# ntampellini/FIRECODE

Measured on AMD Instinct MI355X. Metric: conformer-pair RMSD alignments/s, higher is better.
Workload: dtype f64

## Files before the change

firecode_amd/csrc/fc_items.h:

```cpp
#pragma once

#include <algorithm>
#include <cstdint>
#include <utility>
#include <vector>

#if defined(__HIPCC__) || defined(__CUDACC__)
#define FC_ITEMS_HD __host__ __device__
#else
#define FC_ITEMS_HD
#endif

namespace fc {

FC_ITEMS_HD inline int64_t global_block(int64_t local_block, int64_t rank, int64_t world) {
  return local_block * world + ((local_block & 1) ? (world - 1 - rank) : rank);
}
inline int64_t local_block_count(int64_t n_gblocks, int64_t rank, int64_t world) {
  int64_t n = 0;
  while (global_block(n, rank, world) < n_gblocks) ++n;
  return n;
}

constexpr uint64_t kItemFirstHalf = 1ull << 31, kItemSecondHalf = 1ull << 63;
constexpr int kItemChunkShift = 58, kItemChunkMax = 16;
FC_ITEMS_HD inline int64_t item_tile(uint64_t it) { return (int64_t)(it & 0x7fffffffull); }
FC_ITEMS_HD inline int64_t item_block(uint64_t it) { return (int64_t)((it >> 32) & 0x3ffffffull); }
FC_ITEMS_HD inline int item_blocks(uint64_t it) { return (int)((it >> kItemChunkShift) & 15ull) + 1; }

struct ItemPlan {
  int64_t N = 0, rank = 0, world = 1;
  int64_t row_block = 128, tc = 64;
  int64_t NT = 0, n_lblocks = 0;
  bool halves = false;
  int64_t tail = 0;
  bool real_columns_only = false;
  int64_t chunk = 1;
  bool tail_order = true;
};

template <class F>
inline void item_units(uint64_t it, const ItemPlan &p, F visit) {
  const int64_t jt = item_tile(it), lb = item_block(it), j0 = jt * p.tc, tpb = p.row_block / 16;
  int64_t it_first = 0, it_last = tpb * item_blocks(it);
  if (it & kItemFirstHalf) it_last = tpb / 2;
  if (it & kItemSecondHalf) it_first = tpb / 2;
  const int64_t i0 = global_block(lb, p.rank, p.world) * p.row_block;
  if (i0 >= p.N || j0 + p.tc - 1 <= i0) return;
  for (int64_t t = it_first; t < it_last; ++t) {
    const int64_t ib = global_block(lb + t / tpb, p.rank, p.world) * p.row_block + (t % tpb) * 16;
    if (ib >= p.N) break;
    if (j0 + p.tc - 1 <= ib) break;
    for (int64_t cs = 0; cs < p.tc / 16; ++cs) {
      if (j0 + (cs + 1) * 16 - 1 <= ib) continue;
      if (j0 + cs * 16 >= p.N) continue;
      visit(ib, j0 + cs * 16);
    }
  }
}

inline std::vector<uint64_t> build_items(const ItemPlan &p) {
  std::vector<uint64_t> items;
  if (p.row_block % p.tc != 0) return items;
  const int64_t r = p.row_block / p.tc;
  const int64_t nt = p.real_columns_only ? std::min(p.NT, (p.N + p.tc - 1) / p.tc) : p.NT;
  auto first_tile = [&](int64_t l) { return r * global_block(l, p.rank, p.world); };
  auto n_single = [&](int64_t l) { return std::max<int64_t>(0, nt - first_tile(l)); };
  int64_t n_chunked = 0;
  if (p.chunk > 1) {
    int64_t kept = 0;
    n_chunked = p.n_lblocks;
    while (n_chunked > 0 && kept < (p.tail_order ? 3 : 1) * p.tail) kept += n_single(--n_chunked);
    if (n_chunked < 2) n_chunked = 0;
  }
  const int64_t chunk = std::min<int64_t>(p.chunk, kItemChunkMax);
  for (int64_t l = 0; l < n_chunked; l += chunk) {
    const uint64_t more = (uint64_t)(std::min(chunk, n_chunked - l) - 1);
    for (int64_t jt = first_tile(l); jt < nt; ++jt) items.push_back((more << kItemChunkShift) | ((uint64_t)l << 32) | (uint64_t)jt);
  }
  const size_t single0 = items.size();
  for (int64_t l = n_chunked; l < p.n_lblocks; ++l)
    for (int64_t jt = first_tile(l); jt < nt; ++jt) items.push_back(((uint64_t)l << 32) | (uint64_t)jt);
  if (p.chunk > 1 && p.tail_order) {
    auto cost = [&](uint64_t it) {
      int64_t n = 0;
      item_units(it, p, [&](int64_t, int64_t) { ++n; });
      return n;
    };
    std::vector<std::pair<int64_t, uint64_t>> keyed;
    for (size_t k = single0; k < items.size(); ++k) keyed.emplace_back(-cost(items[k]), items[k]);
    std::stable_sort(keyed.begin(), keyed.end(), [](const auto &a, const auto &b) { return a.first < b.first; });
    for (size_t k = single0; k < items.size(); ++k) items[k] = keyed[k - single0].second;
  }
  if (p.halves && p.tail > 0 && (int64_t)items.size() > 4 * p.tail && (int64_t)(items.size() - single0) >= p.tail) {
    std::vector<uint64_t> halves;
    for (int64_t k = (int64_t)items.size() - p.tail; k < (int64_t)items.size(); ++k) {
      halves.push_back(items[(size_t)k] | kItemFirstHalf);
      halves.push_back(items[(size_t)k] | kItemSecondHalf);
    }
    items.resize(items.size() - (size_t)p.tail);
    items.insert(items.end(), halves.begin(), halves.end());
  }
  return items;
}

}
```

firecode_amd/csrc/fc_kabsch.hip:

```cpp
#include <type_traits>

#include "fc_internal.h"
#include <vector>
#include "fc_kabsch_math.h"

#include <algorithm>
#include <cstdlib>

namespace fc {

__global__ void __launch_bounds__(256)
k_prep(const double *__restrict__ coords, int64_t N, int64_t A_all, const int32_t *__restrict__ sel,
       int64_t A, int center, int64_t Npad, double *__restrict__ Xs, double *__restrict__ G,
       double *__restrict__ Xa, unsigned long long *__restrict__ gmax_bits,
       const int32_t *__restrict__ conf_idx) {
  const int64_t n = (int64_t)blockIdx.x * blockDim.x + threadIdx.x;
  if (n >= Npad) return;
  for (int64_t a = A; a < ((A + 3) & ~(int64_t)3); ++a) {
    Xs[(a * 3 + 0) * Npad + n] = 0.0;
    Xs[(a * 3 + 1) * Npad + n] = 0.0;
    Xs[(a * 3 + 2) * Npad + n] = 0.0;
  }
  if (n >= N) {
    for (int64_t a = 0; a < A; ++a) {
// ... 333 lines not shown
  if (!INV && pi[p] == pj[p]) {
    rmsd[p] = 0.0;
    maxdev[p] = 0.0;
    if (Rout)
      for (int k = 0; k < 9; ++k) Rout[p * 9 + k] = (k % 4 == 0) ? 1.0 : 0.0;
    return;
  }
  pair_exact_aos<INV>(Xa, A, pi[p], pj[p], r, m, Rout ? Rout + p * 9 : nullptr);
  rmsd[p] = r;
  maxdev[p] = m;
}

__global__ void __launch_bounds__(256)
k_matrix_exact(const double *__restrict__ Xs, int64_t N, int64_t Npad, int A,
               double *__restrict__ rmsd, double *__restrict__ maxdev) {
  const int lane = threadIdx.x & 63;
  const int64_t wave = ((int64_t)blockIdx.x * blockDim.x + threadIdx.x) >> 6;
  const int64_t NT = Npad >> 6;
  const int64_t i = wave / NT;
  const int64_t jt = wave % NT;
  if (i >= N) return;
  if (jt * 64 + 63 <= i) return;
  const int64_t j = jt * 64 + lane;
  if (j >= N || j <= i) return;
  double r, m;
  pair_exact(Xs, Npad, A, i, j, r, m);
  rmsd[i * N + j] = r;
  maxdev[i * N + j] = m;
}

__device__ __forceinline__ void push_pairs(uint64_t m, bool may, unsigned i, unsigned j,
                                           uint64_t *__restrict__ pairq, unsigned long long Q,
                                           unsigned long long *__restrict__ counters, int lane) {
  if (m == 0) return;
#ifdef FC_ABLATE_PUSH
  return;
#endif
  unsigned long long base = 0;
  if (lane == 0) base = atomicAdd(&counters[6], (unsigned long long)__popcll(m));
  base = __shfl(base, 0);
  if (may) {
    const unsigned long long slot = base + (unsigned long long)__popcll(m & ((1ull << lane) - 1ull));
    if (slot < Q) pairq[slot] = ((uint64_t)i << 32) | (uint64_t)j;
  }
}

#ifndef FC_REFINE_ROUNDS
#define FC_REFINE_ROUNDS 4
#endif
constexpr int kStagePairs = 48;
constexpr int kStageWords = 24;
constexpr size_t kStageBytes = kStagePairs * 8 + kStageWords * 4 + 8;
constexpr int64_t kCompleteRowChunk = 2;

#ifndef FC_STAGE_PAIRS_F32
#define FC_STAGE_PAIRS_F32 384
#endif
constexpr int kStagePairsF32 = FC_STAGE_PAIRS_F32;
constexpr int kStageWordsF32 = 128;
constexpr size_t kStageBytesF32 = kStagePairsF32 * 8 + kStageWordsF32 * 4 + 16 + 32 * 4;

template <int CAP = kStagePairs>
__device__ __forceinline__ void stage_pairs(uint64_t m, bool may, unsigned i, unsigned j,
                                            uint64_t *__restrict__ sq, unsigned *__restrict__ scnt,
                                            uint64_t *__restrict__ pairq, unsigned long long Q,
                                            unsigned long long *__restrict__ counters, int lane) {
  if (m == 0) return;
#ifdef FC_ABLATE_PUSH
  return;
#endif
#ifdef FC_ABLATE_STAGE
  if (lane == 0) scnt[2] = (unsigned)__popcll(m);
  return;
#endif
  const unsigned n = (unsigned)__popcll(m);
  unsigned base = 0;
  if (lane == 0) base = atomicAdd(scnt, n);
  base = (unsigned)__builtin_amdgcn_readfirstlane((int)base);
  if (base + n <= (unsigned)CAP) {
    if (may) sq[base + (unsigned)__popcll(m & ((1ull << lane) - 1ull))] = ((uint64_t)i << 32) | (uint64_t)j;
  } else {
#ifndef FC_ABLATE_OVERFLOW
    push_pairs(m, may, i, j, pairq, Q, counters, lane);
#endif
  }
}

template <int WCAP>
__device__ __forceinline__ void stage_pairs_wave(uint64_t m, bool may, unsigned i, unsigned j, uint64_t *__restrict__ sq_wave,
                                                 int &n_staged, uint64_t *__restrict__ pairq, unsigned long long Q,
                                                 unsigned long long *__restrict__ counters, int lane) {
  if (m == 0) return;
  const int n = (int)__popcll(m);
  if (n_staged + n <= WCAP) {
    if (may) sq_wave[n_staged + (int)__popcll(m & ((1ull << lane) - 1ull))] = ((uint64_t)i << 32) | (uint64_t)j;
    n_staged += n;
  } else {
    push_pairs(m, may, i, j, pairq, Q, counters, lane);
  }
}

__device__ __forceinline__ void flush_pairs_wave32(const uint32_t *__restrict__ sq_wave, int n_staged, unsigned i0, unsigned j0,
                                                   uint64_t *__restrict__ pairq, unsigned long long Q,
                                                   unsigned long long *__restrict__ counters, int lane) {
  if (n_staged == 0) return;
  unsigned long long base = 0;
// ... 74 lines not shown
        qz = lds[(a * 3 + 2) * 64 + lane];
      } else {
        qx = xq[(int64_t)(a * 3 + 0) * Npad];
        qy = xq[(int64_t)(a * 3 + 1) * Npad];
        qz = xq[(int64_t)(a * 3 + 2) * Npad];
      }
      const double *__restrict__ px = xp + (int64_t)(a * 3 + 0) * Npad;
      const double *__restrict__ py = xp + (int64_t)(a * 3 + 1) * Npad;
      const double *__restrict__ pz = xp + (int64_t)(a * 3 + 2) * Npad;
#pragma unroll
      for (int k = 0; k < TI; ++k) {
        const double x = px[k], y = py[k], z = pz[k];
        acc[k][0] = fma(x, qx, acc[k][0]);
        acc[k][1] = fma(x, qy, acc[k][1]);
        acc[k][2] = fma(x, qz, acc[k][2]);
        acc[k][3] = fma(y, qx, acc[k][3]);
        acc[k][4] = fma(y, qy, acc[k][4]);
        acc[k][5] = fma(y, qz, acc[k][5]);
        acc[k][6] = fma(z, qx, acc[k][6]);
        acc[k][7] = fma(z, qy, acc[k][7]);
        acc[k][8] = fma(z, qz, acc[k][8]);
      }
    }
#pragma unroll
    for (int k = 0; k < TI; ++k) {
      const int64_t i = ib + k;
      const double Gp = G[i];
      bool may = kabsch_may_be_below<ENANT>(acc[k], Gp + Gq, A_thr2);
      may = may && (j > i) && (j < N) && (i < N);
      const uint64_t word = __ballot(may);
      push_pairs(word, may, (unsigned)i, (unsigned)j, pairq, Q, counters, lane);
      if (lane == 0 && i < N) {
        const int64_t lrow = (int64_t)(lb * IB) + (int64_t)it * TI + k;
        bits[lrow * W + jt] = word;
        if (word) {
          const unsigned long long slot = atomicAdd(&counters[4], 1ull);
          cand[slot] = (uint32_t)(lrow * W + jt);
        }
      }
    }
  }
}

typedef double d4_t __attribute__((ext_vector_type(4)));

template <int NW, int MODE = 0, int TC = 64, bool EIG = false, bool ENANT = false>
__global__ void __launch_bounds__(NW * 64, 2)
k_simbits_screen_mfma(const double *__restrict__ Xs, const double *__restrict__ G, int64_t N,
                      int64_t Npad, int A, double A_thr2, int IB, int64_t rank, int64_t world,
                      uint64_t *__restrict__ bits, int64_t W, uint32_t *__restrict__ cand,
                      unsigned long long *__restrict__ counters, uint64_t *__restrict__ pairq,
                      unsigned long long Q, const uint64_t *__restrict__ item_table, unsigned long long n_items,
                      double *__restrict__ rmsd_out = nullptr, const unsigned long long *__restrict__ gate = nullptr,
                      double *__restrict__ maxdev_out = nullptr) {
  static_assert(!EIG || MODE == 2, "EIG: the complete alignments");
  static_assert(!ENANT || MODE == 0, "ENANT: the screen only");
  constexpr bool VALUES = MODE != 0;
  constexpr int NT = MODE == 2 ? 1 : 2;
  static_assert(TC == 64 || ((TC == 32 || TC == 16) && MODE == 2), "column tiles: 64, or 32 / 16 for the complete alignments");
  constexpr int NU = (TC / 16) / NT;
  constexpr int KPR = TC == 64 ? 2 : 4;
  constexpr int SST = 2048 / TC;
  constexpr int CST = TC == 64 ? 256 : 128;
  auto koff = [](int sl) { return TC == 16 ? (sl >> 1) * 384 + (sl & 1) * 64 : sl * (12 * TC); };
  if (gate != nullptr && *gate == 0ull) return;
  extern __shared__ double lds[];
  const int tid = threadIdx.x;
  const int lane = tid & 63;
  const int wv = __builtin_amdgcn_readfirstlane(tid >> 6);
  const int KS = (A + 3) >> 2;
  double *__restrict__ ldsG = lds + (TC == 16 ? ((KS + 1) >> 1) * 384 : KS * 12 * TC);
  uint64_t *__restrict__ stageQ = reinterpret_cast<uint64_t *>(ldsG + TC + IB);
  uint32_t *__restrict__ stageW = reinterpret_cast<uint32_t *>(stageQ + kStagePairs);
  unsigned *__restrict__ stageN = reinterpret_cast<unsigned *>(stageW + kStageWords);
#ifdef FC_TIMELINE
  unsigned long long *tl = MODE == 2 ? reinterpret_cast<unsigned long long *>(bits) : reinterpret_cast<unsigned long long *>(rmsd_out);
  constexpr bool TL = MODE == 0 || MODE == 2;
#endif
  const unsigned long long b = blockIdx.x;
  if (b >= n_items) return;
#ifdef FC_TIMELINE
  if (TL && tl && tid == 0) {
    tl[(size_t)b * 4] = wall_clock64();
    tl[(size_t)b * 4 + 3] = b;
  }
#endif
  int64_t jt, lb;
  int it_first = 0, it_last = IB >> 4;
  if (item_table != nullptr) {
    const uint64_t it = item_table[b];
    lb = item_block(it);
    jt = item_tile(it);
    if constexpr (MODE == 2) it_last = (IB >> 4) * item_blocks(it);
    if (it & kItemFirstHalf) it_last = IB >> 5;
    if (it & kItemSecondHalf) it_first = IB >> 5;
  } else {
    const int64_t NT = Npad / TC;
    jt = (int64_t)(b % (unsigned long long)NT);
    lb = (int64_t)(b / (unsigned long long)NT);
  }
  const int64_t j0 = jt * TC;
  const int64_t i0 = global_block(lb, rank, world) * IB;
  if (i0 >= N) return;
  if (j0 + TC - 1 <= i0) return;
  uint32_t *__restrict__ sq32_wave = reinterpret_cast<uint32_t *>(stageQ) + wv * (kStagePairs * 2 / NW);
  int n_staged32 = 0;
  (void)sq32_wave;
  (void)n_staged32;

  {
    const int n_runs = TC == 64 ? KS * 6 : (TC == 32 ? KS * 3 : ((KS + 1) >> 1) * 3);
    const int cs_l = TC == 64 ? lane >> 4 : lane >> 5, k1_l = TC == 64 ? (lane >> 3) & 1 : (lane >> 3) & 3, c15_l = (lane & 7) * 2;
    for (int q = wv; q < n_runs; q += NW) {
      const int sc = TC == 64 ? q >> 1 : q, kh = TC == 64 ? q & 1 : 0;
      const int sg = sc / 3, c = sc - sg * 3;
      int a = sg * 4 + kh * 2 + k1_l;
      if (TC == 16) {
        a = (sg * 2 + cs_l) * 4 + k1_l;
        a = a < KS * 4 ? a : KS * 4 - 1;
      }
      const double *src = Xs + (int64_t)(a * 3 + c) * Npad + j0 + (TC == 16 ? 0 : cs_l * 16) + c15_l;
      __builtin_amdgcn_global_load_lds((const __attribute__((address_space(1))) void *)src,
                                       (__attribute__((address_space(3))) void *)(lds + q * 128), 16, 0, 0);
    }
    for (int idx = tid; idx < TC + IB; idx += NW * 64) {
      const int64_t g = idx < TC ? j0 + idx : i0 + (idx - TC);
      ldsG[idx] = g < Npad ? G[g] : 0.0;
    }
    if (tid < kStagePairs) stageQ[tid] = ~0ull;
    if (tid < kStageWords) stageW[tid] = ~0u;
    if (tid < 2) stageN[tid] = 0u;
    __syncthreads();
#ifdef FC_TIMELINE
    if (TL && tl && tid == 0) tl[(size_t)b * 4 + 1] = wall_clock64();
#endif
  }
  const int kq = lane >> 4, l15 = lane & 15;
  const int lcol = MODE == 2 ? 4 * (l15 & 3) + (l15 >> 2) : l15;
  const int boff = (kq / KPR) * 128 + (kq % KPR) * 16 + lcol;
  uint16_t *bits16 = reinterpret_cast<uint16_t *>(bits);

  double a0[3], a1[3], a2[3];
  int pre_it = -1;
  const int tpb = IB >> 4;
  auto tile_row = [&](int it_) -> int64_t {
    if constexpr (MODE == 2) {
      const int k = it_ / tpb;
      return global_block(lb + k, rank, world) * IB + (int64_t)(it_ - k * tpb) * 16;
    } else {
      return i0 + (int64_t)it_ * 16;
    }
  };
  auto row_offsets = [&](int it_, unsigned (&vo)[3]) {
    const int64_t ib_ = tile_row(it_);
#pragma unroll
    for (int c = 0; c < 3; ++c) vo[c] = (unsigned)(((int64_t)(kq * 3 + c) * Npad + ib_ + l15) * 8);
  };
  auto fetch_a_at = [&](double (&a)[3], unsigned (&vo)[3], int sx) {
    const int sl = sx < KS ? sx : KS - 1;
    const char *__restrict__ xs_s = reinterpret_cast<const char *>(Xs + (int64_t)sl * 12 * Npad);
#pragma unroll
    for (int c = 0; c < 3; ++c) {
      asm volatile("" : "+v"(vo[c]));
      a[c] = *reinterpret_cast<const double *>(xs_s + vo[c]);
    }
  };

  for (int it = it_first + wv; it < it_last; it += NW) {
    const int64_t ib = tile_row(it);
    if (ib >= N) break;
    if (j0 + TC - 1 <= ib) break;
    const int64_t lrow0 = lb * IB + (int64_t)it * 16;
    double Gp_row = 0.0;
    if constexpr (MODE == 2) Gp_row = G[ib + l15];
    (void)Gp_row;
    unsigned nz = 0;
    unsigned voff[3];
    row_offsets(it, voff);

#pragma unroll 1
    for (int half = 0; half < NU; ++half) {
      const int cs0 = half * NT;
      if (j0 + (cs0 + NT) * 16 - 1 <= ib) {
        if (!VALUES && lane < 16 && ib + lane < N) {
          bits16[((lrow0 + lane) * W + jt) * 4 + cs0] = 0;
          bits16[((lrow0 + lane) * W + jt) * 4 + cs0 + 1] = 0;
        }
        continue;
      }
      if constexpr (MODE == 2) {
        if (j0 + cs0 * 16 >= N) continue;
      }
      d4_t acc[NT][9];

      const double *__restrict__ lb0 = lds + cs0 * SST + boff;
      double b0[NT][3], b1[NT][3];
      const int KSe = KS;
      auto fetch_a = [&](double (&a)[3], int sx) {
        fetch_a_at(a, voff, sx);
      };
      auto fetch_b = [&](double (&b)[NT][3], int sx) {
        const int sl = sx < KS ? sx : KS - 1;
        const double *__restrict__ lb_s = lb0 + koff(sl);
#pragma unroll
        for (int t = 0; t < NT; ++t)
#pragma unroll
          for (int c = 0; c < 3; ++c) b[t][c] = lb_s[c * CST + t * SST];
      };
      auto mma = [&](const double (&a)[3], const double (&b)[NT][3], auto first_) {
        constexpr bool first = decltype(first_)::value;
#pragma unroll
        for (int x = 0; x < 3; ++x)
#pragma unroll
          for (int y = 0; y < 3; ++y)
#pragma unroll
            for (int t = 0; t < NT; ++t) {
              const d4_t c_in = first ? d4_t{0.0, 0.0, 0.0, 0.0} : acc[t][x * 3 + y];
              acc[t][x * 3 + y] = MODE == 2 ? __builtin_amdgcn_mfma_f64_16x16x4f64(b[t][y], a[x], c_in, 0, 0, 0)
                                            : __builtin_amdgcn_mfma_f64_16x16x4f64(a[x], b[t][y], c_in, 0, 0, 0);
            }
      };
      if (pre_it != it) {
        fetch_a_at(a0, voff, 0);
        fetch_a_at(a1, voff, 1);
        fetch_a_at(a2, voff, 2);
      }
      fetch_b(b0, 0);
      fetch_b(b1, 1);
#define FC_KSTEP(AX, BX, U)             \
  if (sgrp + (U) < KSe) {               \
    mma(AX, BX, std::false_type{});     \
    fetch_a(AX, sgrp + (U) + 3);        \
    fetch_b(BX, sgrp + (U) + 2);        \
  }
      mma(a0, b0, std::true_type{});
      fetch_a(a0, 3);
      fetch_b(b0, 2);
      for (int sgrp = 1; sgrp < KSe; sgrp += 6) {
        FC_KSTEP(a1, b1, 0)
        FC_KSTEP(a2, b0, 1)
        FC_KSTEP(a0, b1, 2)
        FC_KSTEP(a1, b0, 3)
        FC_KSTEP(a2, b1, 4)
        FC_KSTEP(a0, b0, 5)
      }
#undef FC_KSTEP
      {
        const bool same_tile = half < NU - 1 && !(MODE == 2 && j0 + (cs0 + NT) * 16 >= N);
        const int nit = same_tile ? it : it + NW;
        bool more = same_tile;
        if (!same_tile && nit < it_last) {
          const int64_t nib = tile_row(nit);
          more = nib < N && !(j0 + TC - 1 <= nib);
        }
        if (more) {
          unsigned vn[3];
          row_offsets(nit, vn);
          fetch_a_at(a0, vn, 0);
          fetch_a_at(a1, vn, 1);
          fetch_a_at(a2, vn, 2);
          pre_it = nit;
        } else {
          pre_it = -1;
        }
      }
      const int n32 = (int)N, ib32 = (int)ib;
#pragma unroll
      for (int t = 0; t < NT; ++t) {
        const int cs = cs0 + t;
        const int j = (int)j0 + cs * 16 + l15;
        const double Gq = ldsG[cs * 16 + l15];
        uint64_t mr[4] = {0, 0, 0, 0};
        if (MODE == 2) {
          const int i = ib32 + l15;
          const int jb = (int)j0 + cs * 16 + 4 * kq;
          const double Gp = Gp_row;
          double nR[4][9];
          bool ok4[4];
          double msdA4[4] = {0.0, 0.0, 0.0, 0.0};
          {
            double B4[4][9], GG[4], Q44[4][4], nq4[4], lam4[4];
#pragma unroll
            for (int r = 0; r < 4; ++r) {
              GG[r] = Gp + ldsG[cs * 16 + 4 * kq + r];
#pragma unroll
              for (int e = 0; e < 9; ++e) B4[r][e] = acc[t][e][r];
            }
            kabsch_quaternion_qcp_lean4(B4, GG, Q44, nq4, ok4, EIG ? lam4 : nullptr);
            if constexpr (EIG) {
              const double k_small = 2e-10 / (double)A;
#pragma unroll
              for (int r = 0; r < 4; ++r) {
                msdA4[r] = GG[r] - 2.0 * lam4[r];
                if (!(msdA4[r] > k_small * GG[r] * GG[r])) ok4[r] = false, msdA4[r] = 0.0;
              }
            }
#pragma unroll
            for (int r = 0; r < 4; ++r) {
              if (!ok4[r]) Q44[r][0] = 1.0, Q44[r][1] = 0.0, Q44[r][2] = 0.0, Q44[r][3] = 0.0, nq4[r] = 1.0;
              neg_rotation_from_raw_quaternion(Q44[r], nq4[r], nR[r]);
            }
// ... 107 lines not shown
          double B9[9];
#pragma unroll
          for (int e = 0; e < 9; ++e) B9[e] = acc[t][e][r];
          if (VALUES) {
            double slope;
            const double lam = kabsch_lambda_max(B9, Gp + Gq, &slope);
            const double msdA = (Gp + Gq) - 2.0 * lam;
            const bool in = (j > i) && (j < n32) && (i < n32);
            if (in) rmsd_out[(int64_t)i * N + j] = sqrt(fmax(msdA, 0.0) / (double)A);
            const bool redo = in && (msdA < A_thr2 || !kabsch_lambda_is_sharp(lam, slope, (double)A, msdA));
            stage_pairs(__ballot(redo), redo, (unsigned)i, (unsigned)j, stageQ, stageN, pairq, Q, counters, lane);
            continue;
          }
          bool may = kabsch_may_be_below<ENANT>(B9, Gp + Gq, A_thr2);
          may = may && (j > i) && (j < n32) && (i < n32);
          mr[r] = __ballot(may);
          if constexpr (MODE == 0)
            stage_pairs_wave32<kStagePairs * 2 / NW>(mr[r], may, (unsigned)i, (unsigned)j, (unsigned)i0, (unsigned)j0, sq32_wave,
                                                     n_staged32, pairq, Q, counters, lane);
          else
            stage_pairs(mr[r], may, (unsigned)i, (unsigned)j, stageQ, stageN, pairq, Q, counters, lane);
        }
        if (!VALUES && lane < 16 && ib32 + lane < n32) {
          const int rr = lane >> 2;
          const uint64_t mine = rr == 0 ? mr[0] : rr == 1 ? mr[1] : rr == 2 ? mr[2] : mr[3];
          const unsigned piece = (unsigned)((mine >> (16 * (lane & 3))) & 0xffffull);
          bits16[((lrow0 + lane) * W + jt) * 4 + cs] = (uint16_t)piece;
          nz |= piece;
        }
      }
    }
    if (!VALUES) {
#ifndef FC_ABLATE_PUSH
      const bool has = lane < 16 && nz != 0;
      const uint64_t mw = __ballot(has);
      if (mw != 0) {
        const unsigned n = (unsigned)__popcll(mw);
        const uint32_t word = (uint32_t)((lrow0 + lane) * W + jt);
        unsigned base = 0;
        if (lane == 0) base = atomicAdd(stageN + 1, n);
        base = (unsigned)__builtin_amdgcn_readfirstlane((int)base);
        const unsigned rank_in = (unsigned)__popcll(mw & ((1ull << lane) - 1ull));
        if (base + n <= (unsigned)kStageWords) {
          if (has) stageW[base + rank_in] = word;
        } else {
          unsigned long long gbase = 0;
          if (lane == 0) gbase = atomicAdd(&counters[4], (unsigned long long)n);
          gbase = __shfl(gbase, 0);
          if (has) cand[gbase + rank_in] = word;
        }
      }
#endif
    }
  }
  if constexpr (MODE == 0) flush_pairs_wave32(sq32_wave, n_staged32, (unsigned)i0, (unsigned)j0, pairq, Q, counters, lane);
  __syncthreads();
#ifdef FC_TIMELINE
  if (TL && tl && tid == 0) tl[(size_t)b * 4 + 2] = wall_clock64();
#endif
  if (wv == 0) {
    if constexpr (MODE != 0) {
      const uint64_t e = lane < kStagePairs ? stageQ[lane] : ~0ull;
      const bool valid = e != ~0ull;
      const uint64_t mv = __ballot(valid);
      if (mv != 0) {
        unsigned long long gbase = 0;
        if (lane == 0) gbase = atomicAdd(&counters[6], (unsigned long long)__popcll(mv));
        gbase = __shfl(gbase, 0);
        if (valid) {
          const unsigned long long slot = gbase + (unsigned long long)__popcll(mv & ((1ull << lane) - 1ull));
          if (slot < Q) pairq[slot] = e;
        }
      }
    }
    if (!VALUES) {
      const uint32_t wq = lane < kStageWords ? stageW[lane] : ~0u;
      const bool valid = wq != ~0u;
      const uint64_t mv = __ballot(valid);
      if (mv != 0) {
        unsigned long long gbase = 0;
        if (lane == 0) gbase = atomicAdd(&counters[4], (unsigned long long)__popcll(mv));
        gbase = __shfl(gbase, 0);
        if (valid) cand[gbase + (unsigned long long)__popcll(mv & ((1ull << lane) - 1ull))] = wq;
      }
    }
  }
}

typedef float f4_t __attribute__((ext_vector_type(4)));

#ifndef FC_F32_WGS
#define FC_F32_WGS 3
#endif
template <int NW, bool BITS = true, bool STAGED = false, int TC = 64, bool ENANT = false>
__global__ void __launch_bounds__(NW * 64, FC_F32_WGS)
k_simbits_screen_mfma_f32(const float *__restrict__ Xsf, const double *__restrict__ G, int64_t N,
                          int64_t Npad, int A, double A_thr2, KabschF32Bounds bd, int IB, int64_t rank,
                          int64_t world, uint64_t *__restrict__ bits, int64_t W, uint32_t *__restrict__ cand,
                          unsigned long long *__restrict__ counters, uint64_t *__restrict__ pairq,
                          unsigned long long Q, const uint64_t *__restrict__ item_table,
                          unsigned long long n_items, const float *__restrict__ sub, KabschF32Bounds bd1,
                          float inv_AS, uint64_t *__restrict__ unitq, int part, int gate) {
  if ((gate == 1 && counters[15] != 0ull) || (gate == 2 && counters[15] == 0ull)) return;
  extern __shared__ double lds_raw[];
  float *__restrict__ lds = reinterpret_cast<float *>(lds_raw);
  static_assert(TC == 64 || (TC == 32 && !BITS && !STAGED), "32-column tiles: lean single-stage launches only");
// ... 1626 lines not shown
        rmsd_out[i * N + j] = r;
        if (maxdev_out) maxdev_out[i * N + j] = m;
      }
    }
  }
}

__global__ void __launch_bounds__(256)
k_scatter_pairs(const uint64_t *__restrict__ pairs, int64_t n_pairs, int64_t N, int64_t W,
                uint64_t *__restrict__ bits) {
  const int64_t p = (int64_t)blockIdx.x * blockDim.x + threadIdx.x;
  if (p >= n_pairs) return;
  const uint64_t e = pairs[p];
  const int64_t i = (int64_t)(e >> 32), j = (int64_t)(e & 0xffffffffull);
  if (i < 0 || j <= i || j >= N) return;
  atomicOr(reinterpret_cast<unsigned long long *>(&bits[i * W + (j >> 6)]), 1ull << (j & 63));
}

static int screen_item_table(fc_ensemble *e, int64_t NT, int64_t n_lblocks, bool halves = true, int64_t tc = 64, int64_t chunk = 0,
                             bool tail_order = true) {
  const int64_t rb_key = (((e->row_block * 2 + (halves ? 1 : 0)) * 128 + tc) * 32 + chunk) * 2 + (tail_order ? 1 : 0);
  if (e->item_key[0] == e->N && e->item_key[1] == e->rank && e->item_key[2] == e->world &&
      e->item_key[3] == rb_key)
    return FC_OK;
  e->item_total = 0;
  e->item_key[0] = e->N; e->item_key[1] = e->rank; e->item_key[2] = e->world; e->item_key[3] = rb_key;
  ItemPlan plan;
  plan.N = e->N; plan.rank = e->rank; plan.world = e->world;
  plan.row_block = e->row_block; plan.tc = tc; plan.NT = NT; plan.n_lblocks = n_lblocks;
  plan.tail = 2 * (int64_t)ctx().n_cu;
  if (const char *v = getenv("FC_SCREEN_TAIL_SLOTS")) plan.tail = std::max<int64_t>(0, std::strtoll(v, nullptr, 10));
  plan.halves = halves && e->row_block == 128 && e->A <= 52;
  plan.real_columns_only = chunk > 0;
  plan.chunk = std::max<int64_t>(1, chunk);
  plan.tail_order = tail_order;
  std::vector<uint64_t> items = build_items(plan);
  if (items.empty() || items.size() >= (1ull << 31)) return FC_OK;
  FC_TRY(e->item_table.reserve(items.size() * sizeof(uint64_t)));
  e->item_host.swap(items);
  FC_TRY(h2d(e->item_table.p, e->item_host.data(), e->item_host.size() * sizeof(uint64_t)));
  e->item_total = (int64_t)e->item_host.size();
  return FC_OK;
}

int prebuild_screen_items(fc_ensemble *e) {
  const int64_t n_lblocks = local_block_count(ceil_div(e->N, e->row_block), e->rank, e->world);
  if (n_lblocks <= 0 || (e->Npad >> 6) == 0) return FC_OK;
  return screen_item_table(e, e->Npad >> 6, n_lblocks, true, 64);
}

template <int NW, int TC, bool EIG>
static int launch_complete_variant(fc_ensemble *e, dim3 grid, size_t lds_m, double A_small, int64_t rb, int64_t rank, int64_t world,
                                   unsigned long long *cnt, const uint64_t *item_table_dev, unsigned long long n_items,
                                   double *rmsd_dev, double *maxdev_dev, uint64_t *timeline_dev) {
  if (lds_m > 64 * 1024) {
    hipError_t err = hipFuncSetAttribute(reinterpret_cast<const void *>(k_simbits_screen_mfma<NW, 2, TC, EIG>),
                                         hipFuncAttributeMaxDynamicSharedMemorySize, (int)lds_m);
    if (err != hipSuccess) return set_error(FC_E_HIP, "hipFuncSetAttribute failed: %s", hipGetErrorString(err));
  }
  hipLaunchKernelGGL((k_simbits_screen_mfma<NW, 2, TC, EIG>), grid, dim3(NW * 64), lds_m, ctx().stream, e->Xs.as<double>(),
                     e->G.as<double>(), e->N, e->Npad, (int)e->A, A_small, (int)rb, rank, world, timeline_dev, e->W, nullptr, cnt,
                     e->pairq.as<uint64_t>(), (unsigned long long)e->pairq_cap, item_table_dev, n_items, rmsd_dev, nullptr,
                     maxdev_dev);
  return FC_OK;
}

int launch_rmsd_values(fc_ensemble *e, double small_rmsd, double *rmsd_dev, double *maxdev_dev, int64_t rank,
                       int64_t world, bool explicit_sum) {
  const int64_t rb = 128;
  const int64_t n_lblocks = local_block_count(ceil_div(e->N, rb), rank, world);
  if (n_lblocks <= 0) return FC_OK;
  const size_t lds_64 = ((size_t)((e->A + 3) / 4) * 4 * 3 * 64 + 64 + (size_t)rb) * sizeof(double) + kStageBytes;
  const size_t lds_32 = ((size_t)((e->A + 3) / 4) * 4 * 3 * 32 + 32 + (size_t)rb) * sizeof(double) + kStageBytes;
  const size_t lds_16 = ((size_t)(((e->A + 3) / 4 + 1) / 2) * 384 + 16 + (size_t)rb) * sizeof(double) + kStageBytes;
  const bool narrow = lds_64 > kLdsLimit && maxdev_dev != nullptr;
  const int64_t tc = !narrow ? 64 : (lds_32 <= kLdsLimit ? 32 : 16);
  const size_t lds_m = tc == 64 ? lds_64 : (tc == 32 ? lds_32 : lds_16);
  const int64_t NT = e->Npad / tc;
  if (lds_m > kLdsLimit || NT == 0)
    return set_error(FC_E_LIMIT, "A=%lld atoms exceed the LDS column tile of the value kernel", (long long)e->A);
  const bool fits32 = (uint64_t)((e->A + 3) / 4 * 4) * 3 * (uint64_t)e->Npad < (1ull << 32) &&
                      96 * (uint64_t)e->Npad < (1ull << 32);
  if (!fits32) return set_error(FC_E_LIMIT, "ensemble too large for 32-bit operand offsets");
  auto *cnt = reinterpret_cast<unsigned long long *>(e->counters.p);
  const bool two_blocks = 2 * lds_m <= kLdsLimit;
  const bool complete = maxdev_dev != nullptr;
  const void *fn = two_blocks ? reinterpret_cast<const void *>(k_simbits_screen_mfma<4, 1>)
                              : reinterpret_cast<const void *>(k_simbits_screen_mfma<8, 1>);
  if (!complete && lds_m > 64 * 1024) {
    hipError_t err = hipFuncSetAttribute(fn, hipFuncAttributeMaxDynamicSharedMemorySize, (int)lds_m);
    if (err != hipSuccess) return set_error(FC_E_HIP, "hipFuncSetAttribute failed: %s", hipGetErrorString(err));
  }
  const double A_small = (double)e->A * small_rmsd * small_rmsd;
  const int64_t saved_rank = e->rank, saved_world = e->world, saved_rb = e->row_block;
  e->rank = rank; e->world = world; e->row_block = rb;
  int64_t chunk = 0;
  bool tail_order = true;
  if (complete) {
    chunk = two_blocks && !narrow ? kCompleteRowChunk : 1;
    if (const char *v = getenv("FC_COMPLETE_ROW_CHUNK")) chunk = std::min<int64_t>(kItemChunkMax, std::max<int64_t>(1, std::strtoll(v, nullptr, 10)));
    if (const char *v = getenv("FC_COMPLETE_TAIL_ORDER")) tail_order = atoi(v) != 0;
  }
  const int rc_tbl = screen_item_table(e, NT, n_lblocks, true, tc, chunk, tail_order);
  e->rank = saved_rank; e->world = saved_world; e->row_block = saved_rb;
  e->item_key[3] = -1;
  if (rc_tbl != FC_OK) return rc_tbl;
  const int compact = e->item_total > 0 ? 1 : 0;
  const unsigned long long n_items =
      compact ? (unsigned long long)e->item_total : (unsigned long long)NT * (unsigned long long)n_lblocks;
  const uint64_t *item_table_dev = compact ? e->item_table.as<uint64_t>() : nullptr;
  if (n_items >= (1ull << 31)) return set_error(FC_E_LIMIT, "too many value-kernel items for one launch");
  const dim3 grid((unsigned)n_items);
  uint64_t *timeline_dev = nullptr;
#ifdef FC_TIMELINE
  static DevBuf tlbuf;
  const bool timeline = complete && getenv("FC_TIMELINE_OUT") != nullptr;
  if (timeline) {
    FC_TRY(tlbuf.reserve(n_items * 4 * sizeof(uint64_t)));
    FC_HIP_TRY(hipMemsetAsync(tlbuf.p, 0, n_items * 4 * sizeof(uint64_t), ctx().stream));
    timeline_dev = tlbuf.as<uint64_t>();
  }
#endif
#define FC_LAUNCH_VALUES(NW_, MODE_)                                                                      \
  hipLaunchKernelGGL((k_simbits_screen_mfma<NW_, MODE_>), grid, dim3(NW_ * 64), lds_m, ctx().stream,      \
                     e->Xs.as<double>(), e->G.as<double>(), e->N, e->Npad, (int)e->A, A_small, (int)rb,   \
                     rank, world, nullptr, e->W, nullptr, cnt, e->pairq.as<uint64_t>(),                   \
                     (unsigned long long)e->pairq_cap, item_table_dev, n_items, rmsd_dev, nullptr, maxdev_dev)
  const char *eig_env = getenv("FC_COMPLETE_EIG");
  const bool eig = complete && !(eig_env && atoi(eig_env) == 0) && !explicit_sum;
#define FC_LAUNCH_COMPLETE(NW_, TC_)                                                                                        \
  FC_TRY((eig ? launch_complete_variant<NW_, TC_, true>(e, grid, lds_m, A_small, rb, rank, world, cnt, item_table_dev, n_items, \
                                                       rmsd_dev, maxdev_dev, timeline_dev)                                 \
              : launch_complete_variant<NW_, TC_, false>(e, grid, lds_m, A_small, rb, rank, world, cnt, item_table_dev,     \
                                                        n_items, rmsd_dev, maxdev_dev, timeline_dev)))
  if (narrow && tc == 32) {
    FC_LAUNCH_COMPLETE(8, 32);
  } else if (narrow) {
    FC_LAUNCH_COMPLETE(8, 16);
  } else if (complete) {
    if (two_blocks) FC_LAUNCH_COMPLETE(4, 64);
    else FC_LAUNCH_COMPLETE(8, 64);
  } else {
    if (two_blocks) FC_LAUNCH_VALUES(4, 1);
    else FC_LAUNCH_VALUES(8, 1);
  }
#undef FC_LAUNCH_COMPLETE
#undef FC_LAUNCH_VALUES
  FC_TRY(check_launch("k_simbits_screen_mfma<values>"));
#ifdef FC_TIMELINE
  if (timeline) {
    std::vector<uint64_t> h(n_items * 4);
    FC_HIP_TRY(hipMemcpyAsync(h.data(), tlbuf.p, h.size() * sizeof(uint64_t), hipMemcpyDeviceToHost, ctx().stream));
    FC_HIP_TRY(hipStreamSynchronize(ctx().stream));
    if (FILE *f = fopen(getenv("FC_TIMELINE_OUT"), "wb")) {
      const uint64_t head[2] = {(uint64_t)n_items, compact ? 1ull : 0ull};
      fwrite(head, sizeof(uint64_t), 2, f);
      fwrite(h.data(), sizeof(uint64_t), h.size(), f);
      if (compact) fwrite(e->item_host.data(), sizeof(uint64_t), e->item_host.size(), f);
      fclose(f);
    }
  }
#endif
  if (ctx().mark_after_screen) (void)hipEventRecord(ctx().mark_after_screen, ctx().stream);
  hipLaunchKernelGGL(k_rmsd_fix_small, dim3((unsigned)(ctx().n_cu * 4)), dim3(256), 0, ctx().stream,
                     e->Xa.as<double>(), (int)e->A, e->N, e->pairq.as<uint64_t>(), cnt,
                     (unsigned long long)e->pairq_cap, rmsd_dev, maxdev_dev);
  return check_launch("k_rmsd_fix_small");
}

__global__ void __launch_bounds__(256)
k_gather_matrix_pairs(const double *__restrict__ rmsd_m, const double *__restrict__ maxdev_m, int64_t N,
                      const int64_t *__restrict__ pi, const int64_t *__restrict__ pj, int64_t P,
                      double *__restrict__ rmsd_out, double *__restrict__ maxdev_out) {
  const int64_t p = (int64_t)blockIdx.x * blockDim.x + threadIdx.x;
  if (p >= P) return;
  int64_t i = pi[p], j = pj[p];
  if (i > j) { const int64_t t = i; i = j; j = t; }
  rmsd_out[p] = rmsd_m[i * N + j];
  maxdev_out[p] = maxdev_m[i * N + j];
}

int launch_gather_matrix_pairs(const double *rmsd_m, const double *maxdev_m, int64_t N, const int64_t *pi_dev,
                               const int64_t *pj_dev, int64_t P, double *rmsd_out, double *maxdev_out) {
  if (P == 0) return FC_OK;
  hipLaunchKernelGGL(k_gather_matrix_pairs, dim3((unsigned)ceil_div(P, 256)), dim3(256), 0, ctx().stream, rmsd_m,
                     maxdev_m, N, pi_dev, pj_dev, P, rmsd_out, maxdev_out);
  return check_launch("k_gather_matrix_pairs");
// ... 443 lines not shown
                       e->Xsf.as<float>(), e->G.as<double>(), e->N, e->Npad, (int)e->A, A_thr2, bd,
                       e->unitq.as<uint64_t>(), cnt, e->pairq.as<uint64_t>(), (unsigned long long)e->pairq_cap);
    FC_TRY(check_launch("k_screen_units_f32"));
    FC_LAUNCH_F32_LEAN(n_items, nullptr, 0, 2, false);
#undef FC_LAUNCH_F32_LEAN
  } else if (e->lean)
    hipLaunchKernelGGL((k_simbits_screen_mfma_f32<4, false, false, 64, ENANT>), mgrid, dim3(256), lds_f, ctx().stream,
                       e->Xsf.as<float>(), e->G.as<double>(), e->N, e->Npad, (int)e->A, A_thr2, bd,
                       (int)e->row_block, e->rank, e->world, e->bits.as<uint64_t>(), e->W,
                       e->cand.as<uint32_t>(), cnt, e->pairq.as<uint64_t>(),
                       (unsigned long long)e->pairq_cap, item_table_dev, n_items, nullptr, bd1, inv_AS, nullptr, 0, 0);
  else
    hipLaunchKernelGGL((k_simbits_screen_mfma_f32<4, true, false, 64, ENANT>), mgrid, dim3(256), lds_f, ctx().stream,
                       e->Xsf.as<float>(), e->G.as<double>(), e->N, e->Npad, (int)e->A, A_thr2, bd,
                       (int)e->row_block, e->rank, e->world, e->bits.as<uint64_t>(), e->W,
                       e->cand.as<uint32_t>(), cnt, e->pairq.as<uint64_t>(),
                       (unsigned long long)e->pairq_cap, item_table_dev, n_items, nullptr, bd1, inv_AS, nullptr, 0, 0);
  return check_launch("k_simbits_screen_mfma_f32");
}
static int launch_f32_screen(fc_ensemble *e, const ScreenPlan &p, int64_t n_lblocks, double A_thr2) {
  return e->enant ? launch_f32_screen_of<true>(e, p, n_lblocks, A_thr2) : launch_f32_screen_of<false>(e, p, n_lblocks, A_thr2);
}

static int launch_fp64_screen(fc_ensemble *e, const ScreenPlan &p, int64_t n_lblocks, double A_thr2,
                              const unsigned long long *gate) {
  const auto fn = e->enant ? (p.fp64_waves == 4 ? k_simbits_screen_mfma<4, 0, 64, false, true> : k_simbits_screen_mfma<8, 0, 64, false, true>)
                            : (p.fp64_waves == 4 ? k_simbits_screen_mfma<4> : k_simbits_screen_mfma<8>);
  const int threads = 64 * p.fp64_waves;
  if (p.lds64 > 64 * 1024) {
    hipError_t err = hipFuncSetAttribute(reinterpret_cast<const void *>(fn), hipFuncAttributeMaxDynamicSharedMemorySize,
                                         (int)p.lds64);
    if (err != hipSuccess)
      return set_error(FC_E_HIP, "hipFuncSetAttribute(LDS=%zu) failed: %s", p.lds64, hipGetErrorString(err));
  }
  if (getenv("FC_DEBUG")) {
    int nb = -1;
    (void)hipOccupancyMaxActiveBlocksPerMultiprocessor(&nb, reinterpret_cast<const void *>(fn), threads, p.lds64);
    fprintf(stderr, "[fc] screen_mfma<%d>: LDS %zu B, occupancy API says %d blocks/CU\n", p.fp64_waves, p.lds64, nb);
  }
  ScreenItems it;
  FC_TRY(screen_items(e, n_lblocks, 64, &it));
  double *dbg = nullptr;
#ifdef FC_TIMELINE
  static DevBuf tlbuf;
  if (p.timeline) {
    FC_TRY(tlbuf.reserve(it.n * 4 * sizeof(unsigned long long)));
    FC_HIP_TRY(hipMemsetAsync(tlbuf.p, 0, it.n * 4 * sizeof(unsigned long long), ctx().stream));
    dbg = tlbuf.as<double>();
  }
#endif
  hipLaunchKernelGGL(fn, dim3((unsigned)it.n), dim3(threads), p.lds64, ctx().stream, e->Xs.as<double>(), e->G.as<double>(), e->N,
                     e->Npad, (int)e->A, A_thr2, (int)e->row_block, e->rank, e->world, e->bits.as<uint64_t>(), e->W,
                     e->cand.as<uint32_t>(), reinterpret_cast<unsigned long long *>(e->counters.p), e->pairq.as<uint64_t>(),
                     (unsigned long long)e->pairq_cap, it.table, it.n, dbg, gate, nullptr);
  FC_TRY(check_launch("k_simbits_screen_mfma"));
#ifdef FC_TIMELINE
  if (p.timeline) {
    std::vector<unsigned long long> h(it.n * 4);
    FC_HIP_TRY(hipMemcpyAsync(h.data(), tlbuf.p, it.n * 4 * sizeof(unsigned long long), hipMemcpyDeviceToHost, ctx().stream));
    FC_HIP_TRY(hipStreamSynchronize(ctx().stream));
    if (FILE *f = fopen(getenv("FC_TIMELINE_OUT"), "wb")) {
      fwrite(h.data(), sizeof(unsigned long long), h.size(), f);
      fclose(f);
    }
  }
#endif
  return FC_OK;
}

static int launch_valu_screen(fc_ensemble *e, const ScreenPlan &p, int64_t n_lblocks, double A_thr2) {
  const auto fn = e->enant ? (p.valu_lds ? k_simbits_screen<true, 8, 4, true> : k_simbits_screen<false, 8, 4, true>)
                            : (p.valu_lds ? k_simbits_screen<true, 8, 4> : k_simbits_screen<false, 8, 4>);
  if (p.lds > 64 * 1024) {
    hipError_t err = hipFuncSetAttribute(reinterpret_cast<const void *>(fn), hipFuncAttributeMaxDynamicSharedMemorySize, (int)p.lds);
    if (err != hipSuccess)
      return set_error(FC_E_HIP, "hipFuncSetAttribute(LDS=%zu) failed: %s", p.lds, hipGetErrorString(err));
  }
  hipLaunchKernelGGL(fn, dim3((unsigned)(e->Npad >> 6), (unsigned)n_lblocks), dim3(256), p.lds, ctx().stream, e->Xs.as<double>(),
                     e->G.as<double>(), e->N, e->Npad, (int)e->A, A_thr2, (int)e->row_block, e->rank, e->world,
                     e->bits.as<uint64_t>(), e->W, e->cand.as<uint32_t>(), reinterpret_cast<unsigned long long *>(e->counters.p),
                     e->pairq.as<uint64_t>(), (unsigned long long)e->pairq_cap);
  return check_launch("k_simbits_screen");
}

int launch_simbits_screen(fc_ensemble *e, double thr2_margin) {
  auto mark_main = []() {
    if (ctx().mark_after_screen) (void)hipEventRecord(ctx().mark_after_screen, ctx().stream);
    if (ctx().after_main_stream && ctx().after_main_event) {
      (void)hipEventRecord(ctx().after_main_event, ctx().stream);
      (void)hipStreamWaitEvent(ctx().after_main_stream, ctx().after_main_event, 0);
      ctx().stream = ctx().after_main_stream;
    }
  };
  if (e->g_max < 0.0) return set_error(FC_E_INVALID, "internal: the screen of an ensemble whose largest G was never set");
  const int64_t n_lblocks = local_block_count(ceil_div(e->N, e->row_block), e->rank, e->world);
  ScreenShape s{e->N, e->Npad, e->A, e->row_block, n_lblocks, e->lean, e->g_max, thr2_margin, -1};
  const ScreenKnobs knobs = screen_knobs();
  ScreenPlan p = plan_screen(s, knobs);
  if (p.needs_h2_model) {
    bool ok = false;
    FC_TRY(h2_model_ok(&ok));
    s.h2_model = ok ? 1 : 0;
    p = plan_screen(s, knobs);
  }
  FC_TRY(screen_plan_error(p, e->row_block));
  if (p.kind == 0) {
    mark_main();
// ... 144 lines not shown
```

Before: 20.21 billion.

## Distribute complete-mode work units across waves by sub-tile with shared-tile mapping

Replaces the per-wave row-tile loop in the complete-alignment (MODE 2) MFMA kernel with an explicit unit iterator. Each unit is a (row tile, 16-column sub-tile) pair that skips dead sub-tiles below the diagonal or past N. A new 'shared' mapping lets all waves of a block split the sub-tiles of one row tile instead of each wave owning whole row tiles. This is meant to balance work across waves near the diagonal and at the tail, and it prefetches the next unit's operands. It adds iterator overhead and is the default only for the wide two-block configuration; an environment variable can override the mapping.

```diff
diff --git a/firecode_amd/csrc/fc_items.h b/firecode_amd/csrc/fc_items.h
--- a/firecode_amd/csrc/fc_items.h
+++ b/firecode_amd/csrc/fc_items.h
@@ -59,6 +59,62 @@
   }
 }
 
+constexpr int kUnitMapRows = 0, kUnitMapShared = 1;
+FC_ITEMS_HD inline int units_first(int64_t ib, int64_t j0) { return ib > j0 ? (int)((ib - j0) >> 4) : 0; }
+FC_ITEMS_HD inline int units_end(int64_t j0, int64_t N, int nu) {
+  const int64_t real = (N - j0 + 15) >> 4;
+  return real < nu ? (int)real : nu;
+}
+template <class RowOf>
+FC_ITEMS_HD inline bool unit_settle(int &it, int &cs, int64_t &ib, int d_it, int it_last, int cs_end, int64_t j0, int64_t N,
+                                    RowOf row_of) {
+  while (cs >= cs_end) {
+    const int over = cs - cs_end;
+    it += d_it;
+    if (it >= it_last) return false;
+    ib = row_of(it);
+    if (ib >= N) return false;
+    const int first = units_first(ib, j0);
+    if (first >= cs_end) return false;
+    cs = first + over;
+  }
+  return true;
+}
+FC_ITEMS_HD inline int unit_step_tiles(int unit_map, int nw) { return unit_map == kUnitMapShared ? 1 : nw; }
+FC_ITEMS_HD inline int unit_step_subtiles(int unit_map, int nw) { return unit_map == kUnitMapShared ? nw : 1; }
+template <class RowOf>
+FC_ITEMS_HD inline bool unit_first_of_wave(int &it, int &cs, int64_t &ib, int unit_map, int nw, int wv, int it_first, int it_last,
+                                           int cs_end, int64_t j0, int64_t N, RowOf row_of) {
+  const int d_it = unit_step_tiles(unit_map, nw);
+  if (cs_end <= 0) return false;
+  it = it_first + (unit_map == kUnitMapShared ? 0 : wv) - d_it;
+  cs = cs_end + (unit_map == kUnitMapShared ? wv : 0);
+  return unit_settle(it, cs, ib, d_it, it_last, cs_end, j0, N, row_of);
+}
+template <class RowOf>
+FC_ITEMS_HD inline bool unit_next_of_wave(int &it, int &cs, int64_t &ib, int unit_map, int nw, int it_last, int cs_end, int64_t j0,
+                                          int64_t N, RowOf row_of) {
+  cs += unit_step_subtiles(unit_map, nw);
+  return unit_settle(it, cs, ib, unit_step_tiles(unit_map, nw), it_last, cs_end, j0, N, row_of);
+}
+
+template <class F>
+inline void item_units_of_wave(uint64_t it, const ItemPlan &p, int unit_map, int nw, int wv, F visit) {
+  const int64_t jt = item_tile(it), lb = item_block(it), j0 = jt * p.tc, tpb = p.row_block / 16;
+  int it_first = 0, it_last = (int)tpb * item_blocks(it);
+  if (it & kItemFirstHalf) it_last = (int)tpb / 2;
+  if (it & kItemSecondHalf) it_first = (int)tpb / 2;
+  const int64_t i0 = global_block(lb, p.rank, p.world) * p.row_block;
+  if (i0 >= p.N || j0 + p.tc - 1 <= i0) return;
+  auto row_of = [&](int t) { return global_block(lb + t / tpb, p.rank, p.world) * p.row_block + (t % tpb) * 16; };
+  const int cs_end = units_end(j0, p.N, (int)(p.tc / 16));
+  int t = 0, cs = 0;
+  int64_t ib = 0;
+  for (bool more = unit_first_of_wave(t, cs, ib, unit_map, nw, wv, it_first, it_last, cs_end, j0, p.N, row_of); more;
+       more = unit_next_of_wave(t, cs, ib, unit_map, nw, it_last, cs_end, j0, p.N, row_of))
+    visit(ib, j0 + (int64_t)cs * 16);
+}
+
 inline std::vector<uint64_t> build_items(const ItemPlan &p) {
   std::vector<uint64_t> items;
   if (p.row_block % p.tc != 0) return items;
diff --git a/firecode_amd/csrc/fc_kabsch.hip b/firecode_amd/csrc/fc_kabsch.hip
--- a/firecode_amd/csrc/fc_kabsch.hip
+++ b/firecode_amd/csrc/fc_kabsch.hip
@@ -409,6 +409,7 @@
 constexpr int kStageWords = 24;
 constexpr size_t kStageBytes = kStagePairs * 8 + kStageWords * 4 + 8;
 constexpr int64_t kCompleteRowChunk = 2;
+constexpr int kCompleteUnitMap[4] = {kUnitMapShared, kUnitMapRows, kUnitMapRows, kUnitMapRows};
 
 #ifndef FC_STAGE_PAIRS_F32
 #define FC_STAGE_PAIRS_F32 384
@@ -589,7 +590,7 @@
                       unsigned long long *__restrict__ counters, uint64_t *__restrict__ pairq,
                       unsigned long long Q, const uint64_t *__restrict__ item_table, unsigned long long n_items,
                       double *__restrict__ rmsd_out = nullptr, const unsigned long long *__restrict__ gate = nullptr,
-                      double *__restrict__ maxdev_out = nullptr) {
+                      double *__restrict__ maxdev_out = nullptr, int unit_map = kUnitMapRows) {
   static_assert(!EIG || MODE == 2, "EIG: the complete alignments");
   static_assert(!ENANT || MODE == 0, "ENANT: the screen only");
   constexpr bool VALUES = MODE != 0;
@@ -688,11 +689,11 @@
       return i0 + (int64_t)it_ * 16;
     }
   };
-  auto row_offsets = [&](int it_, unsigned (&vo)[3]) {
-    const int64_t ib_ = tile_row(it_);
+  auto row_offsets_at = [&](int64_t ib_, unsigned (&vo)[3]) {
 #pragma unroll
     for (int c = 0; c < 3; ++c) vo[c] = (unsigned)(((int64_t)(kq * 3 + c) * Npad + ib_ + l15) * 8);
   };
+  auto row_offsets = [&](int it_, unsigned (&vo)[3]) { row_offsets_at(tile_row(it_), vo); };
   auto fetch_a_at = [&](double (&a)[3], unsigned (&vo)[3], int sx) {
     const int sl = sx < KS ? sx : KS - 1;
     const char *__restrict__ xs_s = reinterpret_cast<const char *>(Xs + (int64_t)sl * 12 * Npad);
@@ -703,30 +704,46 @@
     }
   };
 
-  for (int it = it_first + wv; it < it_last; it += NW) {
-    const int64_t ib = tile_row(it);
-    if (ib >= N) break;
-    if (j0 + TC - 1 <= ib) break;
+  int u_it = 0, u_cs = 0, un_it = 0, un_cs = 0, u_tile = -1;
+  int64_t u_ib = 0, un_ib = 0;
+  bool u_more = false;
+  const int u_end = units_end(j0, N, NU);
+  if constexpr (MODE == 2) u_more = unit_first_of_wave(u_it, u_cs, u_ib, unit_map, NW, wv, it_first, it_last, u_end, j0, N, tile_row);
+  (void)u_tile;
+  (void)un_cs;
+  (void)un_ib;
+  (void)u_end;
+  double Gp_row = 0.0;
+  (void)Gp_row;
+  unsigned voff[3] = {0u, 0u, 0u};
+  if constexpr (MODE == 2) {
+    if (u_more) row_offsets_at(u_ib, voff);
+  }
+  for (int it = MODE == 2 ? u_it : it_first + wv; MODE == 2 ? u_more : it < it_last; it = MODE == 2 ? un_it : it + NW) {
+    const int64_t ib = MODE == 2 ? u_ib : tile_row(it);
+    if constexpr (MODE != 2) {
+      if (ib >= N) break;
+      if (j0 + TC - 1 <= ib) break;
+    }
     const int64_t lrow0 = lb * IB + (int64_t)it * 16;
-    double Gp_row = 0.0;
-    if constexpr (MODE == 2) Gp_row = G[ib + l15];
-    (void)Gp_row;
+    if constexpr (MODE == 2) {
+      if (it != u_tile) Gp_row = G[ib + l15];
+      u_tile = it;
+    }
     unsigned nz = 0;
-    unsigned voff[3];
-    row_offsets(it, voff);
+    if constexpr (MODE != 2) row_offsets(it, voff);
 
 #pragma unroll 1
-    for (int half = 0; half < NU; ++half) {
+    for (int half = MODE == 2 ? u_cs : 0; half < (MODE == 2 ? u_cs + 1 : NU); ++half) {
       const int cs0 = half * NT;
-      if (j0 + (cs0 + NT) * 16 - 1 <= ib) {
-        if (!VALUES && lane < 16 && ib + lane < N) {
-          bits16[((lrow0 + lane) * W + jt) * 4 + cs0] = 0;
-          bits16[((lrow0 + lane) * W + jt) * 4 + cs0 + 1] = 0;
-        }
-        continue;
-      }
-      if constexpr (MODE == 2) {
-        if (j0 + cs0 * 16 >= N) continue;
+      if constexpr (MODE != 2) {
+        if (j0 + (cs0 + NT) * 16 - 1 <= ib) {
+          if (!VALUES && lane < 16 && ib + lane < N) {
+            bits16[((lrow0 + lane) * W + jt) * 4 + cs0] = 0;
+            bits16[((lrow0 + lane) * W + jt) * 4 + cs0 + 1] = 0;
+          }
+          continue;
+        }
       }
       d4_t acc[NT][9];
 
@@ -782,8 +799,18 @@
         FC_KSTEP(a0, b0, 5)
       }
 #undef FC_KSTEP
-      {
-        const bool same_tile = half < NU - 1 && !(MODE == 2 && j0 + (cs0 + NT) * 16 >= N);
+      if constexpr (MODE == 2) {
+        un_it = it, un_cs = u_cs, un_ib = ib;
+        u_more = unit_next_of_wave(un_it, un_cs, un_ib, unit_map, NW, it_last, u_end, j0, N, tile_row);
+        if (u_more) {
+          if (un_it != it) row_offsets_at(un_ib, voff);
+          fetch_a_at(a0, voff, 0);
+          fetch_a_at(a1, voff, 1);
+          fetch_a_at(a2, voff, 2);
+          pre_it = un_it;
+        }
+      } else {
+        const bool same_tile = half < NU - 1;
         const int nit = same_tile ? it : it + NW;
         bool more = same_tile;
         if (!same_tile && nit < it_last) {
@@ -997,6 +1024,7 @@
       }
 #endif
     }
+    if constexpr (MODE == 2) u_cs = un_cs, u_ib = un_ib;
   }
   if constexpr (MODE == 0) flush_pairs_wave32(sq32_wave, n_staged32, (unsigned)i0, (unsigned)j0, pairq, Q, counters, lane);
   __syncthreads();
@@ -2729,7 +2757,7 @@
 template <int NW, int TC, bool EIG>
 static int launch_complete_variant(fc_ensemble *e, dim3 grid, size_t lds_m, double A_small, int64_t rb, int64_t rank, int64_t world,
                                    unsigned long long *cnt, const uint64_t *item_table_dev, unsigned long long n_items,
-                                   double *rmsd_dev, double *maxdev_dev, uint64_t *timeline_dev) {
+                                   double *rmsd_dev, double *maxdev_dev, uint64_t *timeline_dev, int unit_map) {
   if (lds_m > 64 * 1024) {
     hipError_t err = hipFuncSetAttribute(reinterpret_cast<const void *>(k_simbits_screen_mfma<NW, 2, TC, EIG>),
                                          hipFuncAttributeMaxDynamicSharedMemorySize, (int)lds_m);
@@ -2738,7 +2766,7 @@
   hipLaunchKernelGGL((k_simbits_screen_mfma<NW, 2, TC, EIG>), grid, dim3(NW * 64), lds_m, ctx().stream, e->Xs.as<double>(),
                      e->G.as<double>(), e->N, e->Npad, (int)e->A, A_small, (int)rb, rank, world, timeline_dev, e->W, nullptr, cnt,
                      e->pairq.as<uint64_t>(), (unsigned long long)e->pairq_cap, item_table_dev, n_items, rmsd_dev, nullptr,
-                     maxdev_dev);
+                     maxdev_dev, unit_map);
   return FC_OK;
 }
 
@@ -2773,7 +2801,17 @@
   e->rank = rank; e->world = world; e->row_block = rb;
   int64_t chunk = 0;
   bool tail_order = true;
+  int unit_map = kUnitMapRows;
   if (complete) {
+    unit_map = kCompleteUnitMap[!narrow ? (two_blocks ? 0 : 1) : (tc == 32 ? 2 : 3)];
+    if (const char *v = getenv("FC_COMPLETE_UNIT_MAP")) {
+      if (strcmp(v, "shared") == 0) unit_map = kUnitMapShared;
+      else if (strcmp(v, "rows") == 0) unit_map = kUnitMapRows;
+      else {
+        e->rank = saved_rank; e->world = saved_world; e->row_block = saved_rb;
+        return set_error(FC_E_INVALID, "FC_COMPLETE_UNIT_MAP=%s: rows or shared", v);
+      }
+    }
     chunk = two_blocks && !narrow ? kCompleteRowChunk : 1;
     if (const char *v = getenv("FC_COMPLETE_ROW_CHUNK")) chunk = std::min<int64_t>(kItemChunkMax, std::max<int64_t>(1, std::strtoll(v, nullptr, 10)));
     if (const char *v = getenv("FC_COMPLETE_TAIL_ORDER")) tail_order = atoi(v) != 0;
@@ -2807,9 +2845,9 @@
   const bool eig = complete && !(eig_env && atoi(eig_env) == 0) && !explicit_sum;
 #define FC_LAUNCH_COMPLETE(NW_, TC_)                                                                                        \
   FC_TRY((eig ? launch_complete_variant<NW_, TC_, true>(e, grid, lds_m, A_small, rb, rank, world, cnt, item_table_dev, n_items, \
-                                                       rmsd_dev, maxdev_dev, timeline_dev)                                 \
+                                                       rmsd_dev, maxdev_dev, timeline_dev, unit_map)                       \
               : launch_complete_variant<NW_, TC_, false>(e, grid, lds_m, A_small, rb, rank, world, cnt, item_table_dev,     \
-                                                        n_items, rmsd_dev, maxdev_dev, timeline_dev)))
+                                                        n_items, rmsd_dev, maxdev_dev, timeline_dev, unit_map)))
   if (narrow && tc == 32) {
     FC_LAUNCH_COMPLETE(8, 32);
   } else if (narrow) {
@@ -3359,7 +3397,7 @@
   hipLaunchKernelGGL(fn, dim3((unsigned)it.n), dim3(threads), p.lds64, ctx().stream, e->Xs.as<double>(), e->G.as<double>(), e->N,
                      e->Npad, (int)e->A, A_thr2, (int)e->row_block, e->rank, e->world, e->bits.as<uint64_t>(), e->W,
                      e->cand.as<uint32_t>(), reinterpret_cast<unsigned long long *>(e->counters.p), e->pairq.as<uint64_t>(),
-                     (unsigned long long)e->pairq_cap, it.table, it.n, dbg, gate, nullptr);
+                     (unsigned long long)e->pairq_cap, it.table, it.n, dbg, gate, nullptr, kUnitMapRows);
   FC_TRY(check_launch("k_simbits_screen_mfma"));
 #ifdef FC_TIMELINE
   if (p.timeline) {
```

After: 20.40 billion, median of 6. About the same (+1.0%).
